# zyddnys/manga-image-translator

Hardware: AMD Instinct MI355X
Metric: pages/sec end-to-end (detect+OCR+inpaint), 2048x1456 (higher is better)
Workload: dtype f32

## Files before the change

### include/mit_hip.h

```cpp
#ifndef MIT_HIP_H
#define MIT_HIP_H

#include <stdint.h>

#ifdef __cplusplus
extern "C" {
#endif

#define MIT_ABI_VERSION 25
#define MIT_MAX_TAPS 64

enum MitAct {
    MIT_ACT_NONE = 0,
    MIT_ACT_RELU = 1,
    MIT_ACT_LEAKY = 2,
    MIT_ACT_SILU = 3,
    MIT_ACT_SIGMOID = 4,
    MIT_ACT_GELU = 5
};
#define MIT_ACT_POST_FIRST 0x100

enum MitPad {
    MIT_PAD_ZERO = 0,
    MIT_PAD_REFLECT = 1
// ... 125 lines not shown
    double ms, alg_bytes, alg_flops;
} MitProfKernelStat;
int mit_prof_kernels_read(MitProfKernelStat *stats, int max_stats, int *n_stats);

int mit_resize_u8(const uint8_t *src_dev, int B, int H, int W, int C, uint8_t *dst_dev, int dh, int dw, int mode, const int *yidx_dev,
                  const uint16_t *ycoef_dev, const int *xidx_dev, const uint16_t *xcoef_dev, void *stream);
int mit_resample_pil_u8(const uint8_t *src_dev, int B, int H, int W, int C, uint8_t *dst_dev, int n_out, int axis, const int *bounds_dev,
                        const int *coef_dev, int ksize, void *stream);
int mit_bilateral_u8c3(const uint8_t *src_dev, uint8_t *dst_dev, int B, int H, int W, int radius, int ntaps, const int *tap_ofs_dev,
                       const float *tap_w_dev, const float *color_w_dev, void *stream);
int mit_select_u8(const uint8_t *mask_dev, int thr, const uint8_t *a_dev, const uint8_t *b_dev, uint8_t *out_dev, int64_t npix, int C,
                  void *stream);

int mit_rearrange_squares(const uint8_t *page_dev, int H, int W, int transpose, int w, int pw_num, int ph_num, int ph_step, int p_num,
                          uint8_t *sq_dev, void *stream);
int mit_rearrange_stitch(const float *src_dev, int n, int C, int m, int64_t sn, int64_t sc, int64_t sy, int64_t sx, int transpose, int pw_num,
                         int ph_num, int step, int pw, int hh, const int *starts_dev, float *dst_dev, uint8_t *dst_u8_dev, int ops, void *stream);

typedef struct MitRefineWindow {
    int x1, y1, x2, y2;
} MitRefineWindow;
typedef struct MitRefineCand {
    int kind;
    int lo, hi;
    int invert;
} MitRefineCand;
int64_t mit_ctd_refine_workspace_bytes(const MitRefineWindow *windows, int n);
int mit_ctd_refine_hist(const uint8_t *page_dev, const uint8_t *pred_dev, int H, int W, const MitRefineWindow *windows, int n, int *hist_host,
                        void *workspace_dev, int64_t workspace_bytes, void *stream);
int mit_ctd_refine_scores(const uint8_t *page_dev, const uint8_t *pred_dev, int H, int W, const MitRefineWindow *windows, int n,
                          const MitRefineCand *cands_host, uint64_t *sums_host, void *workspace_dev, int64_t workspace_bytes, void *stream);
int mit_ctd_refine_merge(const uint8_t *page_dev, const uint8_t *pred_dev, int H, int W, const MitRefineWindow *windows, int n,
                         const MitRefineCand *order_host, uint8_t *out_dev, void *workspace_dev, int64_t workspace_bytes, void *stream);


typedef struct MitCrfCrop {
    int x, y, w, h;
} MitCrfCrop;

typedef struct MitDilateJob {
    int32_t sx, sy, sw, sh;
    int32_t dx, dy, dw, dh;
    int32_t k, spitch;
    int64_t src_off;
} MitDilateJob;
int mit_mask_dilate_jobs(const uint8_t *src_dev, const MitDilateJob *jobs_host, int n_jobs, uint8_t *dst_dev, int H, int W, int merge,
                         MitDilateJob *jobs_dev, void *stream);
int mit_binarize_u8(uint8_t *buf_dev, int64_t n, void *stream);

int64_t mit_densecrf_workspace_bytes(const MitCrfCrop *crops, int n_crops);
int mit_densecrf_refine(const uint8_t *page_dev, int H, int W, const MitCrfCrop *crops, int n_crops, const uint8_t *mask_dev,
                        uint8_t *out_dev, float *q_dev, float sxy_gauss, float w_gauss, float sxy_bilateral, float srgb_bilateral,
                        float w_bilateral, int iterations, const float *unary_lut_dev, void *workspace_dev, int64_t workspace_bytes,
                        void *stream);


int mit_fft_cols(const float *in_dev, int64_t in_bs, int64_t in_ts, int64_t in_hs, float *out_dev, int64_t out_bs,
                 int64_t out_ts, int64_t out_hs, const float *twiddle_dev, int B, int h, int64_t ncols, int inverse, float scale,
                 void *stream);

int mit_rfft_rows_supported(int w);
int mit_rfft_rows(const float *in_dev, int64_t in_bs, int64_t in_hs, int64_t in_ws, float *out_dev, int64_t out_bs, int64_t out_ts,
                  int64_t out_hs, int64_t out_ks, const float *tables_dev, int B, int h, int w, int C, float scale, void *stream);
int mit_irfft_rows(const float *in_dev, int64_t in_bs, int64_t in_ts, int64_t in_hs, int64_t in_ks, float *out_dev, int64_t out_bs,
                   int64_t out_hs, int64_t out_ws, const float *res_dev, int64_t res_bs, int64_t res_hs, int64_t res_ws,
                   const float *tables_dev, int B, int h, int w, int C, float scale, void *stream);

int mit_lama_prep(const uint8_t *img_dev, const uint8_t *mask_dev, float *out_dev, int B, int H, int W, void *stream);

int mit_lama_prep_padded(const uint8_t *img_dev, const uint8_t *mask_dev, float *out_dev, int B, int H, int W, int pad, int Wp, void *stream);

int mit_lama_mpe_index(const uint8_t *mask_dev, int B, int H, int W, const int *ys_dev, const int *yc_dev,
                       const double *yw_dev, int ymax, const int *xs_dev, const int *xc_dev, const double *xw_dev,
                       int xmax, uint8_t *hole_dev, uint8_t *relpos_dev, uint8_t *direct_dev, void *stream);

int mit_lama_mpe_add(float *x_dev, const uint8_t *mask_dev, const uint8_t *relpos_dev, const uint8_t *direct_dev,
                     const int *ymap_dev, const int *xmap_dev, const float *emb_dev, const float *dirw_dev, float alpha5,
                     float alpha6, int B, int H, int W, void *stream);
int mit_lama_mpe_rows(const uint8_t *mask_dev, const uint8_t *relpos_dev, const uint8_t *direct_dev, const int *ymap_dev,
                      const int *xmap_dev, int32_t *rows_dev, int B, int H, int W, void *stream);

int mit_lama_post(const float *pred_dev, int64_t pred_pixstride, const uint8_t *img_dev, const uint8_t *mask_dev,
                  uint8_t *out_dev, int B, int H, int W, int composite, void *stream);


int mit_aot_prep(const uint8_t *img_dev, const uint8_t *mask_dev, float *out_dev, int B, int H, int W, void *stream);

int mit_aot_gate(const float *in_dev, int64_t in_pixstride, float *out_dev, int64_t out_pixstride, int64_t npix, int C, int relu_nf,
                 void *stream);

int64_t mit_aot_plane_stats_ws(int B, int hw, int C);
int mit_aot_plane_stats(const float *x_dev, int64_t batch_stride, int64_t pixstride, int B, int hw, int C, void *ws_dev, int64_t ws_bytes,
                        float *mean_dev, float *istd_dev, void *stream);

int mit_aot_blend(float *x_dev, int64_t x_bs, int64_t x_ps, const float *fuse_dev, int64_t f_bs, int64_t f_ps, const float *gate_dev,
                  int64_t g_bs, int64_t g_ps, const float *mean_dev, const float *istd_dev, int B, int hw, int C, void *stream);

int mit_aot_post(const float *pre_dev, int64_t pre_pixstride, const uint8_t *img_dev, const uint8_t *mask_dev, uint8_t *out_dev,
                 float *preclip_dev, int B, int H, int W, int composite, void *stream);


int mit_grouped_conv3x3(const float *in_dev, int64_t in_bs, int64_t in_ps, int B, int H, int W, int C, int cpg, int stride, int dilation,
                        const float *w_dev, const float *scale_dev, const float *bias_dev, int act, float alpha, float *out_dev,
                        int64_t out_bs, int64_t out_ps, void *stream);
int64_t mit_grouped_conv3x3_lds_bytes(int stride, int dilation, int cpg);

int64_t mit_se_squeeze_ws(int B, int hw, int C);
int mit_se_squeeze(const float *x_dev, int64_t bs, int64_t ps, int B, int hw, int C, void *ws_dev, int64_t ws_bytes, void *stream);
int mit_se_excite(const void *ws_dev, int B, int hw, int C, const float *w1_dev, const float *b1_dev, const float *w2_dev,
                  const float *b2_dev, float *s_dev, void *stream);
int mit_se_apply(const float *x_dev, int64_t x_bs, int64_t x_ps, const float *s_dev, const float *res_dev, int64_t r_bs, int64_t r_ps,
                 float *out_dev, int64_t o_bs, int64_t o_ps, int B, int hw, int C, int act, void *stream);

int mit_mc2_ffd_pack(const uint8_t *img_dev, int B, int H, int W, int Cin, float sigma, unsigned *pmax_dev, float *out_dev, void *stream);
int mit_mc2_ffd_unpack(const uint8_t *img_dev, int B, int H, int W, int Cin, const unsigned *pmax_dev, const float *noise_dev,
                       int64_t noise_pixstride, uint8_t *plane_dev, uint8_t *bgr_dev, void *stream);
int mit_mc2_gen_in(const uint8_t *plane_dev, int B, int h, int w, float *out_dev, int Hp, int Wp, void *stream);
int mit_mc2_post(const float *pre_dev, int64_t pre_pixstride, int B, int Hp, int Wp, uint8_t *out_dev, int h, int w, void *stream);


int mit_layernorm_rows(const float *in_dev, int64_t in_rowstride, const float *w_dev, const float *b_dev, float *out_dev,
                       int64_t out_rowstride, int64_t rows, int D, float eps, void *stream);
int mit_dwconv7_ln_nhwc(const float *x_dev, int64_t x_pixstride, const float *w_dev, const float *bdw_dev, const float *g_dev,
                        const float *b_dev, float eps, float *out_dev, int64_t out_pixstride, int B, int H, int W, int C, void *stream);
int mit_dwconv7_ln_supported(int C);


int mit_ctd_prep(const uint8_t *img_dev, int B, int H, int W, int nh, int nw, int S, int mode, const int *yidx_dev,
                 const short *ycoef_dev, const int *xidx_dev, const short *xcoef_dev, float *out_dev, void *stream);

int mit_maxpool_nhwc(const float *in_dev, int64_t in_pixstride, float *out_dev, int64_t out_pixstride, int B, int H,
                     int W, int C, int k, void *stream);
int mit_maxpool2d_nhwc(const float *in_dev, float *out_dev, int B, int H, int W, int C, int k, int s, int p, void *stream);
int mit_avgpool2_nhwc(const float *in_dev, int64_t in_pixstride, float *out_dev, int64_t out_pixstride, int B, int Ho,
                      int Wo, int C, void *stream);
int mit_copy_channels(const float *in_dev, int64_t in_pixstride, float *out_dev, int64_t out_pixstride, int64_t npix,
                      int C, void *stream);
int mit_map_to_u8(const float *in_dev, uint8_t *out_dev, int64_t n, int mode, float thr, void *stream);

int mit_axpy(float *out_dev, float a, const float *x_dev, const float *y_dev, int64_t n, void *stream);

int mit_boxes_from_bitmap(const float *pred, const uint8_t *bitmap, int H, int W, int dest_w, int dest_h, int max_candidates,
                          float unclip_ratio, float min_sside, float box_thresh, float min_sside_out, int roll_start,
                          int64_t *boxes_out, float *scores_out, int *n_out);
int64_t mit_boxes_from_bitmap_dev_workspace_bytes(int B, int H, int W, int max_candidates);
int mit_boxes_debug_stamps(void *stamps_dev);
int mit_boxes_from_bitmap_dev(const float *pred_dev, int64_t pred_bs, const uint8_t *bitmap_dev, int64_t bitmap_bs, float thresh, int B, int H, int W, int dest_w, int dest_h,
                              int max_candidates, float unclip_ratio, float min_sside, float box_thresh, float min_sside_out, int roll_start,
                              void *workspace_dev, int64_t workspace_bytes, int64_t *boxes_dev, float *scores_dev, int *counts_dev,
                              int *overflow_dev, void *stream);
int mit_quad_pair_distances(const double *quads, int n, const int32_t *pairs, int m, double *out);
int mit_find_contours_count(const uint8_t *bitmap, int H, int W, int *n_contours, int64_t *n_points);

typedef struct MitMaskRun {
    int32_t y, x0, x1, comp;
} MitMaskRun;
int mit_mask_assign_lines(uint8_t *mask, int H, int W, const int32_t *boxes_xywh, const double *polys, const double *font_size, int M, int V,
                          double keep_threshold, MitMaskRun *runs, int64_t runs_cap, int32_t *assign, int64_t assign_cap, int32_t *line_rects,
                          int64_t *n_runs_out, int32_t *n_comp_out);
int mit_mask_line_crops(const MitMaskRun *runs, int64_t n_runs, const int32_t *assign, const int32_t *jobs, int n_jobs, uint8_t *out,
                        const int64_t *offsets);
int64_t mit_mask_assign_workspace_bytes(int H, int W);
int mit_mask_assign_lines_dev(uint8_t *mask_dev, int H, int W, const int32_t *boxes_xywh_dev, const double *polys_dev,
                              const double *font_size_dev, int M, int V, double keep_threshold, void *ws_dev, int64_t ws_bytes,
                              int32_t *line_rects_dev, void *stream);
int mit_mask_line_crops_dev(const void *ws_dev, int64_t ws_bytes, int H, int W, const int32_t *jobs_dev, const int64_t *offsets_dev,
// ... 150 lines not shown
```

### manga_image_translator_amd/lama.py

```python
from __future__ import annotations

import ctypes as C
import math
from typing import Dict, Optional, Tuple

import numpy as np
import torch

from . import lib as _lib
from . import ops
from .ops import ACT_NONE, ACT_RELU, ACT_SIGMOID, PAD_REFLECT, PAD_ZERO, bn_params, conv_gemm_desc, launch_conv_gemm, tensor_map

LOCAL_C, GLOBAL_C, SPEC_C = 128, 384, 192
MPE_S = 256


def _cat_bn(sd, p1, p2):
    a, b = bn_params(sd, p1), bn_params(sd, p2)
    return tuple(torch.cat([x, y]) for x, y in zip(a[:4], b[:4])) + (a[4],)



def dft_matrices(h: int, w: int):
    wk = w // 2 + 1
# ... 26 lines not shown
    sin_t = np.sin(ang)
    sin_t[0, :] = 0.0
    if w % 2 == 0:
        sin_t[wk - 1, :] = 0.0
    Fi[:, wk:2 * wk] = (-sin_t * sw * a[:, None]).T
    f32 = lambda m: torch.from_numpy(np.ascontiguousarray(m.astype(np.float32)))
    return f32(F1), f32(G2), f32(G2i), f32(Fi)


def rfft_row_tables(w: int) -> torch.Tensor:
    n = w // 2
    a = np.concatenate([2.0 * np.pi * np.arange(n) / n, 2.0 * np.pi * np.arange(n + 1) / w])
    return torch.from_numpy(np.stack([np.cos(a), np.sin(a)], 1).astype(np.float32)).contiguous()



def _area_taps(n_src: int, n_dst: int):
    scale = n_src / n_dst
    rows = []
    for d in range(n_dst):
        if n_dst <= n_src:
            lo, hi = d * scale, (d + 1) * scale
            s0, s1 = int(math.floor(lo)), min(int(math.ceil(hi)), n_src)
            ws = [max(0.0, min(hi, s + 1) - max(lo, s)) / scale for s in range(s0, s1)]
        else:
            inv = n_dst / n_src
            s0 = int(math.floor(d * scale))
            f = (d + 1) - (s0 + 1) * inv
            f = 0.0 if f <= 0 else f - math.floor(f)
            if s0 >= n_src - 1:
                s0, f = n_src - 1, 0.0
            ws = [1.0 - f] + ([f] if f > 0 else [])
        rows.append((s0, ws))
    maxt = max(len(ws) for _, ws in rows)
    start = np.array([s for s, _ in rows], dtype=np.int32)
    cnt = np.array([len(ws) for _, ws in rows], dtype=np.int32)
    wts = np.zeros((n_dst, maxt), dtype=np.float64)
    for d, (_, ws) in enumerate(rows):
        wts[d, :len(ws)] = ws
    return start, cnt, wts, maxt


def _nearest_map(n_dst: int, n_src: int) -> np.ndarray:
    return np.minimum(np.floor(np.arange(n_dst) * (n_src / n_dst)).astype(np.int64), n_src - 1).astype(np.int32)


class _RowPackedStem:

    K, PAD, WIN = 7, 3, 8

    def __init__(self, conv: "ops.Conv2d", weight: torch.Tensor, device):
        Cout, Cin, kh, kw = weight.shape
        if (kh, kw) != (self.K, self.K) or Cin > 4:
            raise ValueError("row-packed stem: 7x7 kernels with <= 4 input channels only")
        w = torch.zeros(self.K, self.WIN, 4, Cout, dtype=torch.float32)
        w[:, :self.K, :Cin] = weight.detach().to(torch.float32).permute(2, 3, 1, 0)
        self.w, self.Kp, self.Np = ops.pack_weight_kn(w.reshape(self.K * self.WIN * 4, Cout), device)
        self.Cout, self.scale, self.bias, self.act = Cout, conv.scale, conv.bias, conv.act

    def padded_shape(self, B, H, W):
        return (B, H + 2 * self.PAD, W + self.WIN, 4)

    def __call__(self, xp: torch.Tensor, out: torch.Tensor, lut: Optional[Tuple[torch.Tensor, torch.Tensor, torch.Tensor]] = None):
        B, Hp, Wp, _ = xp.shape
        H, W = Hp - 2 * self.PAD, Wp - self.WIN
        d = conv_gemm_desc(
            a=xp, NB=B, Hi=Hp, Wi=W, Cin=self.WIN * 4, a_strides=(Hp * Wp * 4, Wp * 4, 4), Ho=H, Wo=W, sy=1, sx=1,
            taps=[(ky, 0, 0) for ky in range(self.K)], pad_mode=PAD_ZERO, w=self.w, ldw=self.Np, Kw=self.Kp, Nw=self.Np,
            N=self.Cout, c=tensor_map(out), scale=self.scale, bias=self.bias, act=self.act)
        if lut is not None:
            rows, t1, t2 = lut
            if rows.dtype != torch.int32 or rows.numel() != B * H * W or t1.shape[1] != self.Cout or t2.shape[1] != self.Cout:
                raise ValueError("row-packed stem: bad lookup tables")
            d.lut_rows, d.lut1, d.lut2, d.lut_ld = rows.data_ptr(), t1.data_ptr(), t2.data_ptr(), self.Cout
        launch_conv_gemm(d)


class _FFC:

    def __init__(self, sd, p, device, winograd=True):
        w_l = torch.cat([sd[p + ".ffc.convl2l.weight"], sd[p + ".ffc.convg2l.weight"]], dim=1)
        self.winograd = winograd
        self._direct = None
        self._direct_src = (sd[p + ".ffc.convl2l.weight"], sd[p + ".ffc.convg2l.weight"], sd[p + ".ffc.convl2g.weight"],
                            bn_params(sd, p + ".bn_l"), device) if winograd else None
        if winograd:
            self.to_l = ops.WinogradConv3x3(w_l, None, pad_mode=PAD_REFLECT, bn=bn_params(sd, p + ".bn_l"), act=ACT_RELU, device=device)
            self.l2g = ops.WinogradConv3x3(sd[p + ".ffc.convl2g.weight"], None, pad_mode=PAD_REFLECT, device=device)
        else:
            self.to_l = ops.Conv2d(w_l, None, padding=1, pad_mode=PAD_REFLECT, bn=bn_params(sd, p + ".bn_l"), act=ACT_RELU,
                                   device=device)
            self.l2g = ops.Conv2d(sd[p + ".ffc.convl2g.weight"], None, padding=1, pad_mode=PAD_REFLECT, device=device)
        st = p + ".ffc.convg2g"
        self.st_in = ops.Conv2d(sd[st + ".conv1.0.weight"], None, bn=bn_params(sd, st + ".conv1.1"), act=ACT_RELU, device=device)
        wf = sd[st + ".fu.conv_layer.weight"].reshape(SPEC_C, 2, SPEC_C, 2)
        wf = wf.permute(3, 2, 1, 0).reshape(2 * SPEC_C, 2 * SPEC_C)
        self.fu_w, self.fu_Kp, self.fu_Np = ops.pack_weight_kn(wf, device)
        g, b, m, v, eps = bn_params(sd, st + ".fu.bn")
        perm = lambda t: t.reshape(SPEC_C, 2).t().reshape(-1)
        sc, bi = ops.fold_bn(perm(g), perm(b), perm(m), perm(v), eps)
        self.fu_scale, self.fu_bias = sc.to(device), bi.to(device)
        self.st_out = ops.Conv2d(sd[st + ".conv2.weight"], None, bn=bn_params(sd, p + ".bn_g"), act=ACT_RELU, device=device)

    def direct(self):
        if not self.winograd:
            return self.to_l, self.l2g
        if self._direct is None:
            w_l2l, w_g2l, w_l2g, bn_l, device = self._direct_src
            self._direct = (ops.Conv2d(torch.cat([w_l2l, w_g2l], dim=1), None, padding=1, pad_mode=PAD_REFLECT, bn=bn_l, act=ACT_RELU,
                                       device=device),
                            ops.Conv2d(w_l2g, None, padding=1, pad_mode=PAD_REFLECT, device=device))
            self._direct_src = None
        return self._direct


def _dilate(m: np.ndarray, r: int) -> np.ndarray:
    p = np.pad(m, ((0, 0), (r, r), (r, r)))
    H, W = m.shape[1:]
    return np.any([p[:, dy:dy + H, dx:dx + W] for dy in range(2 * r + 1) for dx in range(2 * r + 1)], axis=0)


def _pool2(m: np.ndarray) -> np.ndarray:
    m = np.pad(m, ((0, 0), (0, m.shape[1] % 2), (0, m.shape[2] % 2)))
    return m[:, 0::2, 0::2] | m[:, 0::2, 1::2] | m[:, 1::2, 0::2] | m[:, 1::2, 1::2]


def _blocks_any(m: np.ndarray, bh: int, bw: int) -> np.ndarray:
    B, H, W = m.shape
    p = np.pad(m, ((0, 0), (0, -H % bh), (0, -W % bw)))
    return p.reshape(B, p.shape[1] // bh, bh, p.shape[2] // bw, bw).any(axis=(2, 4))


def tail_need_numpy(mask: np.ndarray) -> dict:
    need = np.asarray(mask) >= 127
    out = dict(cells=_blocks_any(need, 8, 32).astype(np.uint8), sub={}, need_out={}, blocks={}, list={}, start={})
    need = _dilate(need, 3)
    for L in (2, 1, 0):
        out["need_out"][L] = need
        sub = _pool2(need)
        blk = _blocks_any(sub, 8, 8)
        out["sub"][L], out["blocks"][L] = sub, blk
        out["list"][L] = np.flatnonzero(blk.reshape(-1)).astype(np.int32)
        out["start"][L] = np.concatenate([[0], np.cumsum(blk.reshape(blk.shape[0], -1).sum(1))]).astype(np.int32)
        need = _dilate(sub, 1)
    return out


class LamaEngine(ops.Engine):

    def __init__(self, gen_sd: Dict[str, torch.Tensor], mpe_sd: Optional[Dict[str, torch.Tensor]] = None,
                 n_blocks: int = 9, device="cuda", fft_h: bool = True, winograd: bool = True, fft_w: bool = True,
                 row_packed_stem: bool = True, masked_tail: bool = True, fold_l2g: bool = True):
        super().__init__(device)
        self.fold_l2g = fold_l2g
        self.masked_tail = masked_tail
        self.winograd = winograd
        self.fft_h = fft_h
        self.fft_w = fft_w
        self.n_blocks = n_blocks
        sd, dev = gen_sd, self.device
        self.stem = ops.Conv2d(sd["model.1.ffc.convl2l.weight"], None, padding=3, pad_mode=PAD_REFLECT,
                               bn=bn_params(sd, "model.1.bn_l"), act=ACT_RELU, device=dev)
        self.stem_packed = _RowPackedStem(self.stem, sd["model.1.ffc.convl2l.weight"], dev) if row_packed_stem else None
        self.down1 = ops.Conv2d(sd["model.2.ffc.convl2l.weight"], None, stride=2, padding=1, pad_mode=PAD_REFLECT,
                                bn=bn_params(sd, "model.2.bn_l"), act=ACT_RELU, device=dev)
        self.down2 = ops.Conv2d(sd["model.3.ffc.convl2l.weight"], None, stride=2, padding=1, pad_mode=PAD_REFLECT,
                                bn=bn_params(sd, "model.3.bn_l"), act=ACT_RELU, device=dev)
        w3 = torch.cat([sd["model.4.ffc.convl2l.weight"], sd["model.4.ffc.convl2g.weight"]], dim=0)
        self.down3 = ops.Conv2d(w3, None, stride=2, padding=1, pad_mode=PAD_REFLECT,
                                bn=_cat_bn(sd, "model.4.bn_l", "model.4.bn_g"), act=ACT_RELU, device=dev)
        self.blocks = [(_FFC(sd, f"model.{5 + i}.conv1", dev, winograd), _FFC(sd, f"model.{5 + i}.conv2", dev, winograd))
                       for i in range(n_blocks)]
        base = 5 + n_blocks + 1
        self.ups = []
        for i in range(3):
            p = base + 3 * i
            self.ups.append(ops.ConvTranspose2d(sd[f"model.{p}.weight"], sd[f"model.{p}.bias"], stride=2, padding=1,
                                                output_padding=1, bn=bn_params(sd, f"model.{p + 1}"), act=ACT_RELU, device=dev))
        p = base + 10
        self.out_conv = ops.ConvSmallCout(sd[f"model.{p}.weight"], sd[f"model.{p}.bias"], pad_mode=PAD_REFLECT,
                                          act=ACT_SIGMOID, device=dev)
        self.mpe = None
        if mpe_sd is not None:
            self.mpe = dict(emb=mpe_sd["rel_pos_emb.weight"].to(torch.float32).to(dev).contiguous(),
                            dirw=mpe_sd["direct_emb.weight"].to(torch.float32).to(dev).contiguous(),
                            alpha5=float(mpe_sd["alpha5"]), alpha6=float(mpe_sd["alpha6"]))
            emb, dirw = self.mpe["emb"].cpu(), self.mpe["dirw"].cpu()
            a5, a6 = torch.tensor(self.mpe["alpha5"], dtype=torch.float32), torch.tensor(self.mpe["alpha6"], dtype=torch.float32)
            t2 = torch.zeros(16, dirw.shape[1], dtype=torch.float32)
            for bits in range(16):
                acc = torch.zeros(dirw.shape[1], dtype=torch.float32)
                for k in range(4):
                    if bits & (1 << k):
                        acc = acc + dirw[k]
                t2[bits] = acc * a6
            self.mpe["lut1"], self.mpe["lut2"] = (emb * a5).contiguous().to(dev), t2.contiguous().to(dev)
        self.planar_tail = 4
        self.mpe_in_stem = True
        self._tw: Dict[int, torch.Tensor] = {}
        self._tw_rows: Dict[int, torch.Tensor] = {}
        self._dft = ops.ShapeCache(4)
        self._mpe_tabs = ops.ShapeCache(4)

    def release_workspace(self):
        super().release_workspace()
        self._dft.clear()
        self._mpe_tabs.clear()

    def _dft_mats(self, h, w):
        return self._dft.get((h, w), lambda: tuple(m.to(self.device) for m in dft_matrices(h, w)))

    def _twiddles(self, h):
        if h not in self._tw:
            ang = 2.0 * np.pi * np.arange(h // 2) / h
            self._tw[h] = torch.from_numpy(np.stack([np.cos(ang), np.sin(ang)], 1).astype(np.float32)).to(self.device).contiguous()
        return self._tw[h]

    def _row_tables(self, w):
        if w not in self._tw_rows:
            self._tw_rows[w] = rfft_row_tables(w).to(self.device)
        return self._tw_rows[w]

    def _fft_h(self, src, dst, dst_strides, B, h, ncols, plane, inverse):
        _lib.check(_lib.load().mit_fft_cols(src.data_ptr(), 2 * plane, plane, ncols, dst.data_ptr(), *dst_strides,
                                            self._twiddles(h).data_ptr(), B, h, ncols, int(inverse), 1.0 / math.sqrt(h),
                                            C.c_void_p(ops.current_stream())), "mit_fft_cols")

    def _mpe_tables(self, H, W):
        def make():
            ys, yc, yw, ymax = _area_taps(H, MPE_S)
            xs, xc, xw, xmax = _area_taps(W, MPE_S)
            dev = self.device
            t = lambda a: torch.from_numpy(np.ascontiguousarray(a)).to(dev)
            return dict(ys=t(ys), yc=t(yc), yw=t(yw), ymax=ymax, xs=t(xs), xc=t(xc), xw=t(xw), xmax=xmax,
                        ymap=t(_nearest_map(H, MPE_S)), xmap=t(_nearest_map(W, MPE_S)))

        return self._mpe_tabs.get((H, W), make)

    _dbg: Optional[dict] = None

    def _dbg_put(self, name: str, t: torch.Tensor):
        if self._dbg is not None and name not in self._dbg:
            self._dbg[name] = t.clone()

    def _fourier_unit(self, ffc: _FFC, t1: torch.Tensor, t2: torch.Tensor, nprod: int = 0):
        if nprod:
            ops.ensure_split(ffc.fu_w)
        B, h, w, Cc = t1.shape
        wk = w // 2 + 1
        plane = h * wk * Cc
        Y = self._buf("fu_Y", B, 2, h, wk, Cc)
        Zf = self._buf("fu_Z", B, 2, h, wk, Cc)
        Z2 = self._buf("fu_Z2", B, 2, h, wk, Cc)
        U = self._buf("fu_U", B, h, 2, wk, Cc)
        one = [(0, 0, 0)]
        fft_half = 0.5 * 2.5 * h * w * math.log2(h * w) * Cc * B
        tag = lambda: _lib.load().mit_prof_tag_next(fft_half)
        lib = _lib.load()
        use_fft_w = self.fft_w and Cc % 4 == 0 and bool(lib.mit_rfft_rows_supported(w))
        use_fft = h >= 2 and (h & (h - 1)) == 0 and h <= 512 and self.fft_h
        if not (use_fft_w and use_fft):
            F1, G2, G2i, Fi = self._dft_mats(h, w)
        st = C.c_void_p(ops.current_stream())
        if use_fft_w:
            _lib.check(lib.mit_rfft_rows(t1.data_ptr(), h * w * Cc, w * Cc, Cc, Y.data_ptr(), 2 * plane, plane, wk * Cc, Cc,
                                         self._row_tables(w).data_ptr(), B, h, w, Cc, 1.0 / math.sqrt(w), st), "mit_rfft_rows")
        else:
            cm = ops.MitTensorMap()
            cm.base, cm.zs1, cm.zs0, cm.bs, cm.ys, cm.xs = Y.data_ptr(), 2 * plane, wk * Cc, 0, plane, Cc
            tag()
            launch_conv_gemm(conv_gemm_desc(
                a=F1, NB=1, Hi=2, Wi=wk, Cin=F1.shape[1], a_strides=(0, wk * F1.shape[1], F1.shape[1]), Ho=2, Wo=wk, sy=1,
                sx=1, taps=one, pad_mode=PAD_ZERO, w=t1, ldw=Cc, Kw=w, Nw=Cc, N=Cc, c=cm, Z=B * h, zdiv=h,
                w_zs=(h * w * Cc, w * Cc)))
        self._dbg_put("fu1_rfft_rows", Y)
        if use_fft:
            self._fft_h(Y, Zf, (2 * plane, plane, wk * Cc), B, h, wk * Cc, plane, False)
        else:
            cm = ops.MitTensorMap()
            cm.base, cm.zs1, cm.zs0, cm.bs, cm.ys, cm.xs = Zf.data_ptr(), 0, 2 * plane, 0, 0, wk * Cc
            tag()
            launch_conv_gemm(conv_gemm_desc(
                a=G2, NB=1, Hi=1, Wi=2 * h, Cin=G2.shape[1], a_strides=(0, 0, G2.shape[1]), Ho=1, Wo=2 * h, sy=1, sx=1, taps=one,
                pad_mode=PAD_ZERO, w=Y, ldw=wk * Cc, Kw=2 * h, Nw=wk * Cc, N=wk * Cc, c=cm, Z=B, zdiv=1 << 30,
                w_zs=(0, 2 * plane)))
        self._dbg_put("fu2_fft_cols", Zf)
        cm = ops.MitTensorMap()
        cm.base, cm.zs1, cm.zs0, cm.bs, cm.ys, cm.xs = Z2.data_ptr(), 0, 0, 2 * plane, wk * Cc, Cc
        cm.nsplit, cm.nhi = Cc, plane
        launch_conv_gemm(conv_gemm_desc(
            a=Zf, NB=B, Hi=h, Wi=wk, Cin=Cc, a_strides=(2 * plane, wk * Cc, Cc), Ho=h, Wo=wk, sy=1, sx=1,
            taps=[(0, 0, 0), (0, 0, plane)], pad_mode=PAD_ZERO, w=ffc.fu_w, ldw=ffc.fu_Np, Kw=ffc.fu_Kp, Nw=ffc.fu_Np,
            N=2 * Cc, c=cm, scale=ffc.fu_scale, bias=ffc.fu_bias, act=ACT_RELU, nprod=nprod))
        self._dbg_put("fu3_spectral_conv", Z2)
        if use_fft:
            self._fft_h(Z2, U, (2 * plane, wk * Cc, 2 * wk * Cc), B, h, wk * Cc, plane, True)
        else:
            cm = ops.MitTensorMap()
            cm.base, cm.zs1, cm.zs0, cm.bs, cm.ys, cm.xs = U.data_ptr(), 0, 2 * plane, 0, wk * Cc, 2 * wk * Cc
            tag()
            launch_conv_gemm(conv_gemm_desc(
                a=G2i, NB=1, Hi=2, Wi=h, Cin=G2i.shape[1], a_strides=(0, h * G2i.shape[1], G2i.shape[1]), Ho=2, Wo=h, sy=1, sx=1, taps=one,
                pad_mode=PAD_ZERO, w=Z2, ldw=wk * Cc, Kw=2 * h, Nw=wk * Cc, N=wk * Cc, c=cm, Z=B, zdiv=1 << 30,
                w_zs=(0, 2 * plane)))
        self._dbg_put("fu4_ifft_cols", U)
        if use_fft_w:
            _lib.check(lib.mit_irfft_rows(U.data_ptr(), 2 * plane, wk * Cc, 2 * wk * Cc, Cc, t2.data_ptr(), h * w * Cc, w * Cc,
                                          Cc, t1.data_ptr(), h * w * Cc, w * Cc, Cc, self._row_tables(w).data_ptr(), B, h, w, Cc,
                                          1.0 / math.sqrt(w), st), "mit_irfft_rows")
            return
        cm = ops.MitTensorMap()
        cm.base, cm.zs1, cm.zs0, cm.bs, cm.ys, cm.xs = t2.data_ptr(), 0, w * Cc, 0, 0, Cc
        pm = ops.MitTensorMap()
        pm.base, pm.zs1, pm.zs0, pm.bs, pm.ys, pm.xs = t1.data_ptr(), 0, w * Cc, 0, 0, Cc
        tag()
        launch_conv_gemm(conv_gemm_desc(
            a=Fi, NB=1, Hi=1, Wi=w, Cin=Fi.shape[1], a_strides=(0, 0, Fi.shape[1]), Ho=1, Wo=w, sy=1, sx=1, taps=one,
            pad_mode=PAD_ZERO, w=U, ldw=Cc, Kw=2 * wk, Nw=Cc, N=Cc, c=cm, post=pm, Z=B * h, zdiv=1 << 30,
            w_zs=(0, 2 * wk * Cc)))

    def _ffc(self, ffc: _FFC, x: torch.Tensor, out: torch.Tensor, residual: Optional[torch.Tensor], nprod: int = 0):
        B, h, w, _ = x.shape
        x_l, x_g = x[..., :LOCAL_C], x[..., LOCAL_C:]
        res_l = None if residual is None else residual[..., :LOCAL_C]
        res_g = None if residual is None else residual[..., LOCAL_C:]
        fold = self.fold_l2g and ffc.winograd and not nprod and self._dbg is None
        P = None if fold else self._buf("ffc_P", B, h, w, GLOBAL_C)
        M_g = None
        if nprod:
            to_l, l2g = ffc.direct()
            to_l(x, out=out[..., :LOCAL_C], post=res_l, nprod=nprod)
            l2g(x_l, out=P, nprod=nprod)
        elif ffc.winograd:
            T = ops.WinogradConv3x3.tiles(B, h, w)
            V = self._buf("wino_v", 36, T, LOCAL_C + GLOBAL_C)
            ffc.to_l.transform_input(x, V)
            self._dbg_put("w1_wino_input", V)
            ffc.to_l.gemm_output(V, self._buf("wino_ml", 36, T, LOCAL_C), out[..., :LOCAL_C], post=res_l)
            self._dbg_put("w2_wino_products_l", self._buf("wino_ml", 36, T, LOCAL_C))
            self._dbg_put("w3_out_local", out[..., :LOCAL_C])
            if fold:
                M_g = ffc.l2g.products(V, self._buf("wino_mg", 36, T, GLOBAL_C))
            else:
                ffc.l2g.gemm_output(V, self._buf("wino_mg", 36, T, GLOBAL_C), P)
            self._dbg_put("w4_wino_products_g", self._buf("wino_mg", 36, T, GLOBAL_C))
            if P is not None:
                self._dbg_put("w5_P", P)
        else:
            ffc.to_l(x, out=out[..., :LOCAL_C], post=res_l)
            ffc.l2g(x_l, out=P)
        t1 = self._buf("ffc_t1", B, h, w, SPEC_C)
        t2 = self._buf("ffc_t2", B, h, w, SPEC_C)
        ffc.st_in(x_g, out=t1, nprod=nprod)
        self._dbg_put("s1_st_in", t1)
        self._fourier_unit(ffc, t1, t2, nprod)
        self._dbg_put("fu5_irfft_rows_plus_t1", t2)
        ffc.st_out(t2, out=out[..., LOCAL_C:], pre=P, wino_pre=M_g, post=res_g, nprod=nprod)
        self._dbg_put("s2_out_global", out[..., LOCAL_C:])

    def _tail_need(self, mask_u8: torch.Tensor):
        B, H, W = mask_u8.shape
        lib = _lib.load()
        cells = self._buf("need_cells", B, H // 8, (W + 31) // 32, dtype=torch.uint8)
        work = self._buf("need_work", int(lib.mit_lama_tail_need_work(B, H, W)), dtype=torch.uint8)
        live = []
        for L in range(3):
            h, w = H >> (3 - L), W >> (3 - L)
            live.append((self._buf(f"need_list{L}", B * ((h + 7) // 8) * ((w + 7) // 8), dtype=torch.int32),
                         self._buf(f"need_start{L}", B + 1, dtype=torch.int32)))
        _lib.check(lib.mit_lama_tail_need(mask_u8.data_ptr(), B, H, W, cells.data_ptr(), live[0][0].data_ptr(), live[0][1].data_ptr(),
                                          live[1][0].data_ptr(), live[1][1].data_ptr(), live[2][0].data_ptr(), live[2][1].data_ptr(),
                                          work.data_ptr(), C.c_void_p(ops.current_stream())), "mit_lama_tail_need")
        return live, cells

    @torch.no_grad()
    def forward(self, img_u8: torch.Tensor, mask_u8: torch.Tensor, taps: Optional[dict] = None, composite: bool = True,
                precision: str = "fp32") -> torch.Tensor:
        if precision not in ("fp32", "bf16"):
            raise ValueError(f"LamaEngine.forward: precision must be 'fp32' or 'bf16' (got {precision!r})")
        nprod = 1 if precision == "bf16" else 0
        if img_u8.dtype != torch.uint8 or mask_u8.dtype != torch.uint8:
            raise TypeError("LamaEngine.forward expects uint8 page and mask tensors")
        if img_u8.dim() != 4 or img_u8.shape[-1] != 3 or tuple(mask_u8.shape) != tuple(img_u8.shape[:3]):
            raise ValueError(f"bad shapes: page {tuple(img_u8.shape)}, mask {tuple(mask_u8.shape)}")
        B, H, W, _ = img_u8.shape
        if H % 8 or W % 8:
            raise ValueError("LamaEngine.forward: H and W must be multiples of 8 (the plugin resizes first, :67-79)")
        img_u8, mask_u8 = img_u8.contiguous(), mask_u8.contiguous()
        lib = _lib.load()
        st = C.c_void_p(ops.current_stream())
        s64 = self._buf("full64", B, H, W, 64)
        packed = self.stem_packed is not None and H > 3 and W > 3
        lut = None
        if self.mpe is not None:
            tb = self._mpe_tables(H, W)
            hole = self._buf("mpe_hole", B, MPE_S, MPE_S, dtype=torch.uint8)
            rel = self._buf("mpe_rel", B, MPE_S, MPE_S, dtype=torch.uint8)
            dr = self._buf("mpe_dir", B, MPE_S, MPE_S, dtype=torch.uint8)
            _lib.check(lib.mit_lama_mpe_index(mask_u8.data_ptr(), B, H, W, tb["ys"].data_ptr(), tb["yc"].data_ptr(),
                                              tb["yw"].data_ptr(), tb["ymax"], tb["xs"].data_ptr(), tb["xc"].data_ptr(),
                                              tb["xw"].data_ptr(), tb["xmax"], hole.data_ptr(), rel.data_ptr(),
                                              dr.data_ptr(), st), "mit_lama_mpe_index")
            if packed and self.mpe_in_stem:
                rows = self._buf("mpe_rows", B * H * W, dtype=torch.int32)
                _lib.check(lib.mit_lama_mpe_rows(mask_u8.data_ptr(), rel.data_ptr(), dr.data_ptr(), tb["ymap"].data_ptr(),
                                                 tb["xmap"].data_ptr(), rows.data_ptr(), B, H, W, st), "mit_lama_mpe_rows")
                lut = (rows, self.mpe["lut1"], self.mpe["lut2"])
        if packed:
            xp = self._buf("in4p", *self.stem_packed.padded_shape(B, H, W))
            _lib.check(lib.mit_lama_prep_padded(img_u8.data_ptr(), mask_u8.data_ptr(), xp.data_ptr(), B, H, W, 3, xp.shape[2], st),
                       "mit_lama_prep_padded")
            self.stem_packed(xp, s64, lut=lut)
        else:
            x4 = self._buf("in4", B, H, W, 4)
            _lib.check(lib.mit_lama_prep(img_u8.data_ptr(), mask_u8.data_ptr(), x4.data_ptr(), B, H, W, st), "mit_lama_prep")
            self.stem(x4, out=s64)
        if self.mpe is not None:
            if lut is None:
                _lib.check(lib.mit_lama_mpe_add(s64.data_ptr(), mask_u8.data_ptr(), rel.data_ptr(), dr.data_ptr(),
                                                tb["ymap"].data_ptr(), tb["xmap"].data_ptr(), self.mpe["emb"].data_ptr(),
                                                self.mpe["dirw"].data_ptr(), self.mpe["alpha5"], self.mpe["alpha6"], B, H, W,
                                                st), "mit_lama_mpe_add")
            if taps is not None:
                taps["mpe_rel"], taps["mpe_dir"], taps["mpe_hole"] = rel.clone(), dr.clone(), hole.clone()
        if taps is not None:
            taps["stem"] = s64.clone()
        d1 = self._buf("d1", B, H // 2, W // 2, 128)
        self.down1(s64, out=d1, nprod=nprod)
        d2 = self._buf("d2", B, H // 4, W // 4, 256)
        self.down2(d1, out=d2, nprod=nprod)
        h, w = H // 8, W // 8
        X = self._buf("X", B, h, w, 512)
        T = self._buf("Xtmp", B, h, w, 512)
        self.down3(d2, out=X, nprod=nprod)
        if taps is not None:
            taps["down"] = X.clone()
        for i, (c1, c2) in enumerate(self.blocks):
            self._ffc(c1, X, T, None, nprod)
            self._ffc(c2, T, X, X, nprod)
            if taps is not None:
                taps[f"block{i}"] = X.clone()
        live = [None, None, None]
        cells = None
        if self.masked_tail and composite and taps is None and self._dbg is None:
            live, cells = self._tail_need(mask_u8)
        u1 = self._buf("d2", B, H // 4, W // 4, 256)
        self.ups[0](X, out=u1, nprod=nprod, live=live[0])
        u2 = self._buf("d1", B, H // 2, W // 2, 128)
        self.ups[1](u1, out=u2, nprod=nprod, live=live[1])
        pred = self._buf("pred", B, H, W, 3)
        if self.planar_tail:
            P = self.planar_tail
            pm = P == 4 and H % 2 == 0 and W % 2 == 0
            u3 = self._buf("full64", 64 // P, B, H, W, P)
            self.ups[2](u2, out=u3, planes=64 // P, parity_major=pm, nprod=nprod, live=live[2])
            self.out_conv(u3, out=pred, parity_major=pm, cells=cells)
        else:
            u3 = self._buf("full64", B, H, W, 64)
            self.ups[2](u2, out=u3, nprod=nprod, live=live[2])
            self.out_conv(u3, out=pred, cells=cells)
        if taps is not None:
            taps["pred"] = pred.clone()
        out = torch.empty(B, H, W, 3, dtype=torch.uint8, device=self.device)
        _lib.check(lib.mit_lama_post(pred.data_ptr(), 3, img_u8.data_ptr(), mask_u8.data_ptr(), out.data_ptr(), B, H, W,
                                     int(composite), st), "mit_lama_post")
        return out

    def flops_per_page(self, H: int, W: int) -> float:
        px = H * W
        conv = 2.0 * px * (49 * 4 * 64 + 49 * 64 * 3)
        conv += 2.0 * (px / 4) * 9 * 64 * 128 + 2.0 * (px / 16) * 9 * 128 * 256 + 2.0 * (px / 64) * 9 * 256 * 512
        per_ffc = 2.0 * (px / 64) * (9 * (128 * 128 + 384 * 128 + 128 * 384) + 384 * 192 + 192 * 384)
        per_ffc += 2.0 * (px / 64) * ((W // 8 // 2 + 1) / (W // 8)) * 384 * 384
        conv += per_ffc * 2 * self.n_blocks
        conv += 2.0 * (px / 64) * 9 * 512 * 256 + 2.0 * (px / 16) * 9 * 256 * 128 + 2.0 * (px / 4) * 9 * 128 * 64
        return conv
```

Baseline: 47.17.

## Run each LaMa FFC layer through one native call with an optional side stream

Adds a native entry point that runs a whole FFC layer (Winograd local conv, l2g, spectral FFT chain, st_out) from one cached descriptor, in place of many Python-side kernel launches. When two_queues is enabled, the spectral chain runs on a side HIP stream concurrently with the 3x3 chain, with event fork and join. two_queues defaults to False, so by default only the host-side launch batching and descriptor caching apply. The cache keys on data pointers and adds native code paths that must match the Python fallback exactly.

After: 47.22 (median of 3 runs). No clear change (+0.1%).

```diff
diff --git a/include/mit_hip.h b/include/mit_hip.h
--- a/include/mit_hip.h
+++ b/include/mit_hip.h
@@ -231,6 +231,74 @@
 
 int mit_lama_post(const float *pred_dev, int64_t pred_pixstride, const uint8_t *img_dev, const uint8_t *mask_dev,
                   uint8_t *out_dev, int B, int H, int W, int composite, void *stream);
+
+typedef struct MitWino43In {
+    const float *x_dev;
+    int64_t x_bs, x_ys, x_xs;
+    float *v_dev;
+    int32_t B, H, W, C;
+    int32_t pad_mode, _pad;
+} MitWino43In;
+typedef struct MitWino43Out {
+    const float *m_dev;
+    float *y_dev;
+    int64_t y_bs, y_ys, y_xs;
+    const float *post_dev;
+    int64_t p_bs, p_ys, p_xs;
+    const float *scale_dev, *bias_dev;
+    int32_t B, H, W, N;
+    int32_t act;
+    float alpha;
+} MitWino43Out;
+typedef struct MitFftCols {
+    const float *in_dev;
+    int64_t in_bs, in_ts, in_hs;
+    float *out_dev;
+    int64_t out_bs, out_ts, out_hs;
+    const float *twiddle_dev;
+    int64_t ncols;
+    int32_t B, h;
+    int32_t inverse;
+    float scale;
+} MitFftCols;
+typedef struct MitRfftRows {
+    const float *in_dev;
+    int64_t in_bs, in_hs, in_ws;
+    float *out_dev;
+    int64_t out_bs, out_ts, out_hs, out_ks;
+    const float *tables_dev;
+    int32_t B, h, w, C;
+    float scale;
+    int32_t _pad;
+} MitRfftRows;
+typedef struct MitIrfftRows {
+    const float *in_dev;
+    int64_t in_bs, in_ts, in_hs, in_ks;
+    float *out_dev;
+    int64_t out_bs, out_hs, out_ws;
+    const float *res_dev;
+    int64_t res_bs, res_hs, res_ws;
+    const float *tables_dev;
+    int32_t B, h, w, C;
+    float scale;
+    int32_t _pad;
+} MitIrfftRows;
+typedef struct MitLamaFfcLayer {
+    MitWino43In wino_in;
+    MitConvGemm to_l;
+    MitWino43Out wino_out;
+    MitConvGemm l2g;
+    MitConvGemm st_in;
+    MitRfftRows rfft;
+    MitFftCols fft_h;
+    MitConvGemm spec;
+    MitFftCols ifft_h;
+    MitIrfftRows irfft;
+    MitConvGemm st_out;
+    int32_t two_queues;
+    int32_t _pad;
+} MitLamaFfcLayer;
+int mit_lama_ffc_layer(const MitLamaFfcLayer *layer, void *stream);
 
 
 int mit_aot_prep(const uint8_t *img_dev, const uint8_t *mask_dev, float *out_dev, int B, int H, int W, void *stream);
diff --git a/manga_image_translator_amd/csrc/lama_ffc.hip b/manga_image_translator_amd/csrc/lama_ffc.hip
--- /dev/null
+++ b/manga_image_translator_amd/csrc/lama_ffc.hip
@@ -0,0 +1,135 @@
+#include <hip/hip_runtime.h>
+#include <mutex>
+#include "../../include/mit_hip.h"
+#include "common.h"
+
+namespace {
+
+struct SideQueue {
+    std::mutex mu;
+    hipStream_t stream = nullptr;
+    hipEvent_t fork = nullptr, done = nullptr;
+};
+
+constexpr int kMaxDevices = 16;
+
+struct SideQueues {
+    SideQueue q[kMaxDevices];
+    ~SideQueues() {
+        for (auto &s : q) {
+            if (s.fork) (void)hipEventDestroy(s.fork);
+            if (s.done) (void)hipEventDestroy(s.done);
+            if (s.stream) (void)hipStreamDestroy(s.stream);
+        }
+    }
+};
+
+SideQueues &side_queues() {
+    static SideQueues s;
+    return s;
+}
+
+int ensure_side_queue(SideQueue &q) {
+    if (q.stream) return 0;
+    hipStream_t st = nullptr;
+    hipEvent_t fork = nullptr, done = nullptr;
+    hipError_t e = hipStreamCreateWithFlags(&st, hipStreamNonBlocking);
+    if (e == hipSuccess) e = hipEventCreateWithFlags(&fork, hipEventDisableTiming);
+    if (e == hipSuccess) e = hipEventCreateWithFlags(&done, hipEventDisableTiming);
+    if (e != hipSuccess) {
+        if (done) (void)hipEventDestroy(done);
+        if (fork) (void)hipEventDestroy(fork);
+        if (st) (void)hipStreamDestroy(st);
+        return mit_set_error("mit_lama_ffc_layer: cannot create the side stream: %s", hipGetErrorString(e));
+    }
+    q.stream = st;
+    q.fork = fork;
+    q.done = done;
+    return 0;
+}
+
+int run_wino_in(const MitWino43In &a, void *s) {
+    return mit_wino43_input(a.x_dev, a.x_bs, a.x_ys, a.x_xs, a.v_dev, a.B, a.H, a.W, a.C, a.pad_mode, s);
+}
+int run_wino_out(const MitWino43Out &a, void *s) {
+    return mit_wino43_output(a.m_dev, a.y_dev, a.y_bs, a.y_ys, a.y_xs, a.post_dev, a.p_bs, a.p_ys, a.p_xs, a.scale_dev, a.bias_dev, a.B, a.H, a.W,
+                             a.N, a.act, a.alpha, s);
+}
+int run_fft_cols(const MitFftCols &a, void *s) {
+    return mit_fft_cols(a.in_dev, a.in_bs, a.in_ts, a.in_hs, a.out_dev, a.out_bs, a.out_ts, a.out_hs, a.twiddle_dev, a.B, a.h, a.ncols, a.inverse,
+                        a.scale, s);
+}
+int run_rfft(const MitRfftRows &a, void *s) {
+    return mit_rfft_rows(a.in_dev, a.in_bs, a.in_hs, a.in_ws, a.out_dev, a.out_bs, a.out_ts, a.out_hs, a.out_ks, a.tables_dev, a.B, a.h, a.w, a.C,
+                         a.scale, s);
+}
+int run_irfft(const MitIrfftRows &a, void *s) {
+    return mit_irfft_rows(a.in_dev, a.in_bs, a.in_ts, a.in_hs, a.in_ks, a.out_dev, a.out_bs, a.out_hs, a.out_ws, a.res_dev, a.res_bs, a.res_hs,
+                          a.res_ws, a.tables_dev, a.B, a.h, a.w, a.C, a.scale, s);
+}
+
+int conv3x3_chain(const MitLamaFfcLayer &d, void *s) {
+    if (run_wino_in(d.wino_in, s)) return 1;
+    if (mit_conv_gemm(&d.to_l, s)) return 1;
+    if (run_wino_out(d.wino_out, s)) return 1;
+    return mit_conv_gemm(&d.l2g, s);
+}
+
+int spectral_chain(const MitLamaFfcLayer &d, void *s) {
+    if (mit_conv_gemm(&d.st_in, s)) return 1;
+    if (run_rfft(d.rfft, s)) return 1;
+    if (run_fft_cols(d.fft_h, s)) return 1;
+    if (mit_conv_gemm(&d.spec, s)) return 1;
+    if (run_fft_cols(d.ifft_h, s)) return 1;
+    return run_irfft(d.irfft, s);
+}
+
+const char *null_stage(const MitLamaFfcLayer &d) {
+    if (!d.wino_in.x_dev || !d.wino_in.v_dev) return "wino_in";
+    if (!d.to_l.a || !d.to_l.w || !d.to_l.c.base) return "to_l";
+    if (!d.wino_out.m_dev || !d.wino_out.y_dev) return "wino_out";
+    if (!d.l2g.a || !d.l2g.w || !d.l2g.c.base) return "l2g";
+    if (!d.st_in.a || !d.st_in.w || !d.st_in.c.base) return "st_in";
+    if (!d.rfft.in_dev || !d.rfft.out_dev || !d.rfft.tables_dev) return "rfft";
+    if (!d.fft_h.in_dev || !d.fft_h.out_dev || !d.fft_h.twiddle_dev) return "fft_h";
+    if (!d.spec.a || !d.spec.w || !d.spec.c.base) return "spec";
+    if (!d.ifft_h.in_dev || !d.ifft_h.out_dev || !d.ifft_h.twiddle_dev) return "ifft_h";
+    if (!d.irfft.in_dev || !d.irfft.out_dev || !d.irfft.tables_dev) return "irfft";
+    if (!d.st_out.a || !d.st_out.w || !d.st_out.c.base) return "st_out";
+    return nullptr;
+}
+
+}
+
+extern "C" int mit_lama_ffc_layer(const MitLamaFfcLayer *layer, void *stream) {
+    if (!layer) return mit_set_error("mit_lama_ffc_layer: null descriptor");
+    const MitLamaFfcLayer &d = *layer;
+    if (const char *which = null_stage(d)) return mit_set_error("mit_lama_ffc_layer: null operand in stage %s", which);
+
+    if (!d.two_queues || mit_probe_on()) {
+        if (conv3x3_chain(d, stream)) return 1;
+        if (spectral_chain(d, stream)) return 1;
+        return mit_conv_gemm(&d.st_out, stream);
+    }
+
+    int dev = 0;
+    MIT_CHECK_HIP(hipGetDevice(&dev));
+    if (dev < 0 || dev >= kMaxDevices) return mit_set_error("mit_lama_ffc_layer: device %d is beyond the %d side queues", dev, kMaxDevices);
+    SideQueue &q = side_queues().q[dev];
+    std::lock_guard<std::mutex> lk(q.mu);
+    if (ensure_side_queue(q)) return 1;
+    hipStream_t main = (hipStream_t)stream;
+
+    MIT_CHECK_HIP(hipEventRecord(q.fork, main));
+    MIT_CHECK_HIP(hipStreamWaitEvent(q.stream, q.fork, 0));
+    int rc = spectral_chain(d, q.stream);
+    hipError_t e_done = hipEventRecord(q.done, q.stream);
+    if (!rc) rc = conv3x3_chain(d, stream);
+    hipError_t e_join = e_done == hipSuccess ? hipStreamWaitEvent(main, q.done, 0) : e_done;
+    if (e_join != hipSuccess) {
+        (void)hipStreamSynchronize(q.stream);
+        if (!rc) rc = mit_set_error("mit_lama_ffc_layer: cannot join the side stream: %s", hipGetErrorString(e_join));
+    }
+    if (rc) return 1;
+    return mit_conv_gemm(&d.st_out, stream);
+}
diff --git a/manga_image_translator_amd/lama.py b/manga_image_translator_amd/lama.py
--- a/manga_image_translator_amd/lama.py
+++ b/manga_image_translator_amd/lama.py
@@ -132,6 +132,7 @@
         w_l = torch.cat([sd[p + ".ffc.convl2l.weight"], sd[p + ".ffc.convg2l.weight"]], dim=1)
         self.winograd = winograd
         self._direct = None
+        self.native_descs = ops.ShapeCache(4)
         self._direct_src = (sd[p + ".ffc.convl2l.weight"], sd[p + ".ffc.convg2l.weight"], sd[p + ".ffc.convl2g.weight"],
                             bn_params(sd, p + ".bn_l"), device) if winograd else None
         if winograd:
@@ -200,8 +201,10 @@
 
     def __init__(self, gen_sd: Dict[str, torch.Tensor], mpe_sd: Optional[Dict[str, torch.Tensor]] = None,
                  n_blocks: int = 9, device="cuda", fft_h: bool = True, winograd: bool = True, fft_w: bool = True,
-                 row_packed_stem: bool = True, masked_tail: bool = True, fold_l2g: bool = True):
+                 row_packed_stem: bool = True, masked_tail: bool = True, fold_l2g: bool = True, two_queues: bool = False):
         super().__init__(device)
+        self.two_queues = two_queues
+        self._serial = False
         self.fold_l2g = fold_l2g
         self.masked_tail = masked_tail
         self.winograd = winograd
@@ -256,6 +259,9 @@
         super().release_workspace()
         self._dft.clear()
         self._mpe_tabs.clear()
+        for pair in self.blocks:
+            for ffc in pair:
+                ffc.native_descs.clear()
 
     def _dft_mats(self, h, w):
         return self._dft.get((h, w), lambda: tuple(m.to(self.device) for m in dft_matrices(h, w)))
@@ -292,6 +298,17 @@
     def _dbg_put(self, name: str, t: torch.Tensor):
         if self._dbg is not None and name not in self._dbg:
             self._dbg[name] = t.clone()
+
+    @staticmethod
+    def _spectral_conv_desc(ffc: _FFC, Zf: torch.Tensor, Z2: torch.Tensor, B: int, h: int, wk: int, Cc: int, nprod: int = 0):
+        plane = h * wk * Cc
+        cm = ops.MitTensorMap()
+        cm.base, cm.zs1, cm.zs0, cm.bs, cm.ys, cm.xs = Z2.data_ptr(), 0, 0, 2 * plane, wk * Cc, Cc
+        cm.nsplit, cm.nhi = Cc, plane
+        return conv_gemm_desc(
+            a=Zf, NB=B, Hi=h, Wi=wk, Cin=Cc, a_strides=(2 * plane, wk * Cc, Cc), Ho=h, Wo=wk, sy=1, sx=1,
+            taps=[(0, 0, 0), (0, 0, plane)], pad_mode=PAD_ZERO, w=ffc.fu_w, ldw=ffc.fu_Np, Kw=ffc.fu_Kp, Nw=ffc.fu_Np,
+            N=2 * Cc, c=cm, scale=ffc.fu_scale, bias=ffc.fu_bias, act=ACT_RELU, nprod=nprod)
 
     def _fourier_unit(self, ffc: _FFC, t1: torch.Tensor, t2: torch.Tensor, nprod: int = 0):
         if nprod:
@@ -335,13 +352,7 @@
                 pad_mode=PAD_ZERO, w=Y, ldw=wk * Cc, Kw=2 * h, Nw=wk * Cc, N=wk * Cc, c=cm, Z=B, zdiv=1 << 30,
                 w_zs=(0, 2 * plane)))
         self._dbg_put("fu2_fft_cols", Zf)
-        cm = ops.MitTensorMap()
-        cm.base, cm.zs1, cm.zs0, cm.bs, cm.ys, cm.xs = Z2.data_ptr(), 0, 0, 2 * plane, wk * Cc, Cc
-        cm.nsplit, cm.nhi = Cc, plane
-        launch_conv_gemm(conv_gemm_desc(
-            a=Zf, NB=B, Hi=h, Wi=wk, Cin=Cc, a_strides=(2 * plane, wk * Cc, Cc), Ho=h, Wo=wk, sy=1, sx=1,
-            taps=[(0, 0, 0), (0, 0, plane)], pad_mode=PAD_ZERO, w=ffc.fu_w, ldw=ffc.fu_Np, Kw=ffc.fu_Kp, Nw=ffc.fu_Np,
-            N=2 * Cc, c=cm, scale=ffc.fu_scale, bias=ffc.fu_bias, act=ACT_RELU, nprod=nprod))
+        launch_conv_gemm(self._spectral_conv_desc(ffc, Zf, Z2, B, h, wk, Cc, nprod))
         self._dbg_put("fu3_spectral_conv", Z2)
         if use_fft:
             self._fft_h(Z2, U, (2 * plane, wk * Cc, 2 * wk * Cc), B, h, wk * Cc, plane, True)
@@ -369,8 +380,77 @@
             pad_mode=PAD_ZERO, w=U, ldw=Cc, Kw=2 * wk, Nw=Cc, N=Cc, c=cm, post=pm, Z=B * h, zdiv=1 << 30,
             w_zs=(0, 2 * wk * Cc)))
 
+    def ffc_form(self, ffc: _FFC, h: int, w: int, nprod: int = 0) -> str:
+        if nprod or self._dbg is not None or not (ffc.winograd and self.fold_l2g and self.fft_h and self.fft_w):
+            return "python"
+        if not (h >= 2 and (h & (h - 1)) == 0 and h <= 512 and _lib.load().mit_rfft_rows_supported(w)):
+            return "python"
+        return "native"
+
+    def _ffc_native(self, ffc: _FFC, x: torch.Tensor, out: torch.Tensor, residual: Optional[torch.Tensor]):
+        B, h, w, _ = x.shape
+        Cc, wk = SPEC_C, w // 2 + 1
+        plane = h * wk * Cc
+        T = ops.WinogradConv3x3.tiles(B, h, w)
+        V = self._buf("wino_v", 36, T, LOCAL_C + GLOBAL_C)
+        Ml = self._buf("wino_ml", 36, T, LOCAL_C)
+        Mg = self._buf("wino_mg", 36, T, GLOBAL_C)
+        t1 = self._buf("ffc_t1", B, h, w, Cc)
+        t2 = self._buf("ffc_t2", B, h, w, Cc)
+        Y = self._buf("fu_Y", B, 2, h, wk, Cc)
+        Zf = self._buf("fu_Z", B, 2, h, wk, Cc)
+        Z2 = self._buf("fu_Z2", B, 2, h, wk, Cc)
+        U = self._buf("fu_U", B, h, 2, wk, Cc)
+        operands = (x, out, V, Ml, Mg, t1, t2, Y, Zf, Z2, U)
+        key = (B, h, w, x.stride(), out.stride(), None if residual is None else (residual.data_ptr(), residual.stride()),
+               *(t.data_ptr() for t in operands))
+
+        def make():
+            x_l, x_g = x[..., :LOCAL_C], x[..., LOCAL_C:]
+            out_l, out_g = out[..., :LOCAL_C], out[..., LOCAL_C:]
+            res_l = None if residual is None else residual[..., :LOCAL_C]
+            res_g = None if residual is None else residual[..., LOCAL_C:]
+            tw, rows = self._twiddles(h), self._row_tables(w)
+            L = _lib.MitLamaFfcLayer()
+            a = L.wino_in
+            a.x_dev, a.x_bs, a.x_ys, a.x_xs, a.v_dev = x.data_ptr(), x.stride(0), x.stride(1), x.stride(2), V.data_ptr()
+            a.B, a.H, a.W, a.C, a.pad_mode = B, h, w, x.shape[3], ffc.to_l.pad_mode
+            L.to_l = ffc.to_l.gemm_desc(V, Ml)
+            a = L.wino_out
+            a.m_dev, a.y_dev, a.y_bs, a.y_ys, a.y_xs = Ml.data_ptr(), out_l.data_ptr(), out_l.stride(0), out_l.stride(1), out_l.stride(2)
+            if res_l is not None:
+                a.post_dev, a.p_bs, a.p_ys, a.p_xs = res_l.data_ptr(), res_l.stride(0), res_l.stride(1), res_l.stride(2)
+            a.scale_dev, a.bias_dev = ops._ptr(ffc.to_l.scale), ops._ptr(ffc.to_l.bias)
+            a.B, a.H, a.W, a.N, a.act, a.alpha = B, h, w, LOCAL_C, ffc.to_l.act, ffc.to_l.alpha
+            L.l2g = ffc.l2g.gemm_desc(V, Mg)
+            L.st_in = ffc.st_in.desc(x_g, t1)
+            a = L.rfft
+            a.in_dev, a.in_bs, a.in_hs, a.in_ws = t1.data_ptr(), h * w * Cc, w * Cc, Cc
+            a.out_dev, a.out_bs, a.out_ts, a.out_hs, a.out_ks = Y.data_ptr(), 2 * plane, plane, wk * Cc, Cc
+            a.tables_dev, a.B, a.h, a.w, a.C, a.scale = rows.data_ptr(), B, h, w, Cc, 1.0 / math.sqrt(w)
+            for a, src, dst, strides, inverse in ((L.fft_h, Y, Zf, (2 * plane, plane, wk * Cc), 0),
+                                                  (L.ifft_h, Z2, U, (2 * plane, wk * Cc, 2 * wk * Cc), 1)):
+                a.in_dev, a.in_bs, a.in_ts, a.in_hs = src.data_ptr(), 2 * plane, plane, wk * Cc
+                a.out_dev, (a.out_bs, a.out_ts, a.out_hs) = dst.data_ptr(), strides
+                a.twiddle_dev, a.ncols, a.B, a.h, a.inverse, a.scale = tw.data_ptr(), wk * Cc, B, h, inverse, 1.0 / math.sqrt(h)
+            L.spec = self._spectral_conv_desc(ffc, Zf, Z2, B, h, wk, Cc)
+            a = L.irfft
+            a.in_dev, a.in_bs, a.in_ts, a.in_hs, a.in_ks = U.data_ptr(), 2 * plane, wk * Cc, 2 * wk * Cc, Cc
+            a.out_dev, a.out_bs, a.out_hs, a.out_ws = t2.data_ptr(), h * w * Cc, w * Cc, Cc
+            a.res_dev, a.res_bs, a.res_hs, a.res_ws = t1.data_ptr(), h * w * Cc, w * Cc, Cc
+            a.tables_dev, a.B, a.h, a.w, a.C, a.scale = rows.data_ptr(), B, h, w, Cc, 1.0 / math.sqrt(w)
+            blocks = ops.full_block_list(B, h, w, x.device)
+            L.st_out = ffc.st_out.desc(t2, out_g, None, res_g, 0, Mg, live=blocks)
+            return L, (tw, rows, blocks)
+
+        L, _keep = ffc.native_descs.get(key, make)
+        L.two_queues = 0 if self._serial else int(self.two_queues)
+        _lib.check(_lib.load().mit_lama_ffc_layer(C.byref(L), C.c_void_p(ops.current_stream())), "mit_lama_ffc_layer")
+
     def _ffc(self, ffc: _FFC, x: torch.Tensor, out: torch.Tensor, residual: Optional[torch.Tensor], nprod: int = 0):
         B, h, w, _ = x.shape
+        if self.ffc_form(ffc, h, w, nprod) == "native":
+            return self._ffc_native(ffc, x, out, residual)
         x_l, x_g = x[..., :LOCAL_C], x[..., LOCAL_C:]
         res_l = None if residual is None else residual[..., :LOCAL_C]
         res_g = None if residual is None else residual[..., LOCAL_C:]
@@ -485,6 +565,7 @@
         self.down3(d2, out=X, nprod=nprod)
         if taps is not None:
             taps["down"] = X.clone()
+        self._serial = taps is not None
         for i, (c1, c2) in enumerate(self.blocks):
             self._ffc(c1, X, T, None, nprod)
             self._ffc(c2, T, X, X, nprod)
```
